# microsoft/mgl

Measured on AMD Instinct MI355X. Metric: GCUPS (+ aligned reads/s) for 150 bp short-read batch, higher is better.
Workload: dtype int16; 1 GPU; BASELINE.json configs[1]: 10000000 Illumina-style 150 bp reads x 256-base reference windows, affine-gap SW, full matrix, GATK params (200,-150,260,11), SOFTCLIP, scores+offset+CIGAR for every pair; pairs_total=10000000, pairs_per_gpu=10000000, target_len=256, query_len=150, input=ascii, parallelism=1 GPU, steps_in_flight=1

## Files before the change

mgl_amd/csrc/sw_capi.cpp:

```cpp
#include "../../include/mgl_sw.h"

#include <hip/hip_runtime.h>

#include <algorithm>
#include <chrono>
#include <cstdint>
#include <cstdio>
#include <functional>
#include <future>
#include <cstring>
#include <mutex>
#include <string>
#include <vector>

#include "sw_ctx_access.h"
#include "sw_device.h"

using namespace mgl_sw_dev;

static_assert(sizeof(mgl_sw_score) == sizeof(Score), "mgl_sw_score layout");

namespace {

constexpr int64_t kDefaultWorkspace = 4ll << 30;
// ... 890 lines not shown
            da.uni_ql = max_ql;
            da.tb = pt.tb;
            da.tb_stride_words = pt.stride;
            da.rec = pt.rec;
            da.scratch = pt.lane ? static_cast<unsigned char *>(ctx->bnd[h].p) : (use_scratch || coop_waves || strip16) ? static_cast<unsigned char *>(ctx->scratch.p) : nullptr;
            da.diag = nullptr;
            da.matrix = d_matrix;
            da.code = d_code;
            da.matrix_lds_offset = 0;
            da.score_only = score_only ? 1 : 0;
            da.grouped = pt.lane && auto_group ? 1 : 0;
            da.strip_k = strip16 ? strip_k : 0;
            da.strip_passes = strip16 ? strip_passes : 0;
            {
                const char *const sce = getenv("MGL_SW_DEBUG_STRIP_CODES");
                da.strip_codes = strip16 && strip_k > 0 && !(sce && atoi(sce) == 0) && strip16_lds_bytes_codes(max_ql, strip_waves) <= 64 * 1024 ? 1 : 0;
            }
            da.fold_k = P.fold.k;
            da.fold_bm = P.fold.bm;
            da.fold_bx = P.fold.bx;
            {
                const char *const wse = getenv("MGL_SW_DEBUG_WALK_STAGED");
                da.walk_staged = wse && atoi(wse) != 0 ? 1 : 0;
            }
            da.lane_slots = 0;
            da.tile_ctr = nullptr;
            da.grid_fault = nullptr;
            da.gate = nullptr;
            da.gate_dev = nullptr;
            da.gate_failed = nullptr;
            da.gate_timeout_ticks = 0;
            if (pt.lane && (lane_ck || da.grouped)) {
                da.lane_slots = (int)std::min<int64_t>(lane_slots - (side && n_parts > 1 ? std::min<int64_t>(side_reserve, lane_slots / 2) : 0), (pt.count + 127) / 128);
                if (ctx->cur_gate && !hooks) {
                    da.gate = ctx->cur_gate;
                    da.gate_dev = ctx->cur_gate_dev;
                    da.gate_failed = reinterpret_cast<int32_t *>(const_cast<int64_t *>(ctx->cur_gate) + 1);
                    da.gate_timeout_ticks = 100000000u;
                    if (const char *const gte = getenv("MGL_SW_DEBUG_GATE_TIMEOUT_TICKS")) da.gate_timeout_ticks = (unsigned)atoll(gte);
                }
                if ((pt.count + 127) / 128 > da.lane_slots) {
                    da.tile_ctr = static_cast<unsigned *>(ctx->tile_ctr.p) + (size_t)(ctx->tile_seq++ % kTileCounters) * kTileCounterWords;
                    void *fault_dev = nullptr;
                    HIP_TRY(ctx, hipHostGetDevicePointer(&fault_dev, ctx->pin_fault, 0));
                    da.grid_fault = static_cast<int32_t *>(fault_dev);
                }
// ... 2029 lines not shown
```

mgl_amd/csrc/sw_device.h:

```cpp
#ifndef MGL_SW_DEVICE_H
#define MGL_SW_DEVICE_H

#include <hip/hip_runtime.h>
#include <stddef.h>
#include <stdint.h>

namespace mgl_sw_dev {

constexpr int NEG_INF = -0x40000000;
constexpr int OS_SOFTCLIP = 1, OS_INDEL = 2, OS_LEAD_ID = 4, OS_IGNORE = 8;
constexpr int ERR_CIGAR_OVERFLOW = 2;
constexpr int ERR_DEVICE = 4;
constexpr int MATRIX_DIM = 32;

struct Score {
    int32_t mqe, mqe_t, max, max_t, max_q, seg_length;
};

struct DpRecord {
    int32_t mqe, mqe_t, max, max_t, max_q, seg;
    int32_t g_tail;
    int32_t sps;
};

// ... 17 lines not shown
};

struct DpArgs {
    SeqSet t, q;
    int64_t first;
    int64_t count;
    int match, mismatch, gopen, gext, strategy;
    int sps_cap;
    int uni_tl, uni_ql;
    uint32_t *tb;
    int64_t tb_stride_words;
    DpRecord *rec;
    unsigned char *scratch;
    unsigned long long *diag;
    const int8_t *matrix;
    const uint8_t *code;
    int matrix_lds_offset;
    int score_only;
    int grouped;
    int strip_k;
    int strip_passes;
    int strip_codes;
    int lane_slots;
    unsigned *tile_ctr;
    int32_t *grid_fault;
    const int64_t *gate;
    int64_t *gate_dev;
    int32_t *gate_failed;
    unsigned gate_timeout_ticks;
    const int32_t *tile_order;
    const int64_t *slot_off;
    int fold_k, fold_bm, fold_bx;
    int walk_staged;
};

struct TbArgs {
    SeqSet t, q;
    int64_t first, count;
    int strategy;
    const uint32_t *tb;
    int64_t tb_stride_words;
    int packed16;
    int rows_per_stripe;
    int uni_ql;
    const DpRecord *rec;
    int32_t *offset;
// ... 243 lines not shown
```

mgl_amd/csrc/sw_dp16_lane_ck.hip:

```cpp
#include <hip/hip_runtime.h>
#include <stdint.h>
#include <stdio.h>
#include <stdlib.h>
#include <string.h>

#include <type_traits>

#include "sw_device.h"
#include "sw_lane_cell.h"
#include "sw_traceback.h"

#ifndef MGL_CK_ABLATE
#define MGL_CK_ABLATE 0
#endif
#if (MGL_CK_ABLATE != 0 || defined(MGL_CK_PHASES) || defined(MGL_CK_TRACE)) && !defined(MGL_VARIANT_BUILD)
#error "MGL_CK_ABLATE / MGL_CK_PHASES are measurement builds (scripts/build_variant.sh defines MGL_VARIANT_BUILD): never the shipped library"
#endif

#ifdef MGL_CK_PHASES
__device__ unsigned long long mgl_ck_phase_ticks[16];
#define CK_PHASE(k)                                                                                    \
    do {                                                                                               \
        const unsigned long long now_ = __builtin_amdgcn_s_memtime();                                  \
        if (lane == 0) atomicAdd(&mgl_ck_phase_ticks[k], now_ - phase_t0);                             \
// ... 52 lines not shown
#pragma unroll
        for (int k = 0; k < W / 4 + 2; ++k) e[k] = (d[k + 2] & by2) | (d[k] & ~by2);
#pragma unroll
        for (int k = 0; k < W / 4 + 1; ++k) w[k] = (e[k + 1] & by1) | (e[k] & ~by1);
        return s & 3u;
    }
};

struct WaveMem {
    uint2 *bnd;
    uint2 *mid;
    unsigned *ck;
    uint4 *blk;
    const uint2 *rows;
    const unsigned *cku;
    const uint32_t *blku;
    const unsigned *seq;
    unsigned mid_off, t_off, lane;
    template <class T>
    __device__ __forceinline__ static T at32(const void *base, unsigned byte_off) { return *reinterpret_cast<const T *>(static_cast<const char *>(base) + byte_off); }
    __device__ __forceinline__ uint2 row16(int m, int ql, int j) const
    {
        return at32<uint2>(rows, 8u * ((m & 1) ? mid_off + (unsigned)(((m >> 1) * ql + j - 1) * 64) + lane : (unsigned)(((m >> 1) * (ql + 1) + j) * 64) + lane));
    }
    __device__ __forceinline__ unsigned qblock(int blk4, int half) const { return at32<unsigned>(seq, 4u * ((unsigned)((2 * blk4 + half) * 64) + lane)); }
    __device__ __forceinline__ unsigned tblock(int blk4, int half) const { return at32<unsigned>(seq, 4u * (t_off + (unsigned)((2 * blk4 + half) * 64) + lane)); }
    __device__ __forceinline__ unsigned flags(int cc, int r4) const { return at32<unsigned>(blku, 4u * ((unsigned)(cc * 256 + r4) + 4u * lane)); }
};

struct WinShift {
    unsigned t, q;
};
struct PathWalk {
    int I, J, pi, pj, n, seg;
    int hc;
    int mode;
    char state;
    bool done;
    bool stuck;
    SeqBlocks ts, qs;
    CigarWriter cw;

    __device__ __forceinline__ void take(char next, int step)
    {
        if (next == state) {
            seg += step;
// ... 165 lines not shown
        }
        return n;
    }
    static constexpr int VB = 4;
    __device__ __forceinline__ WinShift win64_load(const WaveMem &wm, int half, int tblocks, int qblocks, const BlockGeom &g, unsigned (&tw)[17], unsigned (&qw)[17]) const
    {
        WinShift sh;
        if (g.direct) {
            sh.t = ts.window<64>(I, g.tl, tw);
            sh.q = qs.window<64>(J, g.ql, qw);
            return sh;
        }
        const int dt = (I - 64) >> 2, dq = (J - 64) >> 2;
#pragma unroll
        for (int k = 0; k < 17; ++k) {
            tw[k] = wm.tblock(min(max(dt + k, 0), tblocks - 1), half);
            qw[k] = wm.qblock(min(max(dq + k, 0), qblocks - 1), half);
        }
        sh.t = (unsigned)(I - 64) & 3u;
        sh.q = (unsigned)(J - 64) & 3u;
        return sh;
    }
    __device__ __forceinline__ int stretch_to(int m) const { return min(I - max((((I - 1) >> 4) - m) << 4, 0), J); }
    __device__ __forceinline__ void grid_load(const WaveMem &wm, int ql, unsigned (&w)[VB]) const
    {
#pragma unroll
        for (int m = 0; m < VB; ++m) {
            const int L = stretch_to(m), ie = I - L, je = J - L;
            w[m] = wm.row16(ie >> 4, ql, max(je, 1)).x;
        }
    }
    __device__ __forceinline__ bool verify_apply(const unsigned (&tw)[17], const unsigned (&qw)[17], const WinShift sh, const unsigned (&w)[VB], int half,
                                                 const BlockGeom &g)
    {
        if (!can_verify()) return false;
        const unsigned st = sh.t, sq = sh.q;
        unsigned long long differ = 0;
#pragma unroll
        for (int k = 0; k < 16; ++k) {
            const unsigned tt = __builtin_amdgcn_alignbyte(tw[k + 1], tw[k], st);
            const unsigned nz = nonzero_bytes((g.codes ? tt << 3 : tt) ^ __builtin_amdgcn_alignbyte(qw[k + 1], qw[k], sq)) >> 7;
            const unsigned nib = ((nz * 0x08040201u) >> 24) & 0xfu;
            differ |= (unsigned long long)nib << (4 * (15 - k));
        }
        int took = 0, h_at = hc;
        bool all = true;
#pragma unroll
        for (int m = 0; m < VB; ++m) {
            const int L = stretch_to(m), ie = I - L, je = J - L;
            const int he = ie == 0 ? border(je, g.gopen, g.gext, g.indel)
                         : je == 0 ? border(ie, g.gopen, g.gext, g.indel)
                                   : (half ? hi16(w[m]) : lo16(w[m])) - (ie + je) * g.gext - g.base;
// ... 1 lines not shown
            const bool ok = hc - he == L * g.match + __popcll(differ & in) * (g.mismatch - g.match);
            took = ok ? L : took;
            h_at = ok ? he : h_at;
            all = all && ok;
        }
        stuck = !all;
        if (took > 0) {
            take('M', took);
            I -= took;
            J -= took;
            hc = h_at;
            pi = I;
            pj = J;
            done = !(I > 0 && J > 0);
        }
        return all && !done;
    }
    __device__ __forceinline__ int edge_len() const
    {
        if (done || mode != 0 || !stuck) return 0;
        const int lc = J - ((J - 1) & ~(CK - 1));
        return J > CK && lc < stretch_to(0) ? lc : 0;
    }
    __device__ __forceinline__ unsigned edge_load(const WaveMem &wm, int nb, int lc) const
    {
        const int r0 = I - lc - 1, b = (J - 1) / CK;
        return WaveMem::at32<unsigned>(wm.cku, 4u * ((unsigned)((((r0 >> 5) * (nb - 1) + (b - 1)) * 64 + 2 * (r0 & (R - 1))) * 64) + wm.lane));
    }
    __device__ __forceinline__ bool edge_apply(const unsigned w, const unsigned (&tw)[5], const unsigned (&qw)[5], const WinShift sh, int lc, int half,
                                               const BlockGeom &g)
    {
        if (lc == 0) return false;
        const int ie = I - lc, je = J - lc;
        const int he = (half ? hi16(w) : lo16(w)) - (ie + je) * g.gext - g.base;
        if (hc - he != lc * g.match + mismatches(tw, qw, sh, lc, g.codes) * (g.mismatch - g.match)) return false;
        take('M', lc);
        I = ie;
        J = je;
        hc = he;
        pi = I;
        pj = J;
        return true;
    }
    __device__ __forceinline__ void finish(const TbArgs &a, const DpRecord *rp, int64_t o)
    {
        int off;
        if (a.strategy == OS_SOFTCLIP) {
            cw.push_front(state, seg);
            if (J > 0) cw.push_front('S', J);
// ... 31 lines not shown

constexpr int ROW_KEY_MAX_QL = 65536;
__device__ __forceinline__ int row_pref(const int tl, const int ql, const int j)
{
    const int d = abs(tl - j);
    const int nearer = max(min(ql, tl + d - 1) - max(1, tl - d + 1) + 1, 0);
    return ql - 1 - nearer - ((j > tl && tl - d >= 1) ? 1 : 0);
}
__device__ __forceinline__ int row_col(const int tl, const int ql, const int pref)
{
    const int r = ql - 1 - pref;
    if (tl > ql) return ql - r;
    const int m = min(tl - 1, ql - tl);
    if (r <= 2 * m) return (r & 1) ? tl - ((r + 1) >> 1) : tl + (r >> 1);
    return tl - 1 > m ? tl - (r - m) : tl + (r - m);
}

enum : int {
    NOT_LAST = 0,
    LAST_ROW_KEYS = 1,
    LAST_ROW_STORED = 2,
};

template <int LAST, int CODES>
__device__ __forceinline__ void ck_strip(const int k, const int tl, const int ql, const int nb, const WaveMem &wm, const unsigned *qst, const unsigned *tst,
                                         const LaneConsts &c, const int gopen, const int gext, const int base, const bool indel, int &bestA,
                                         int &bestA_i, int &bestB, int &bestB_i, int &keyA, int &keyB, unsigned &corner)
{
    const int i0 = k * R;
    unsigned h[R], f[R], t[R];
#pragma unroll
    for (int r4 = 0; r4 < R / 4; ++r4) {
        const unsigned ta = tst[(size_t)(2 * ((i0 >> 2) + r4)) * 64], tb = tst[(size_t)(2 * ((i0 >> 2) + r4) + 1) * 64];
        t[4 * r4 + 0] = __builtin_amdgcn_perm(tb, ta, 0x0c040c00u) | (CODES ? CODE_SEL : 0u);
        t[4 * r4 + 1] = __builtin_amdgcn_perm(tb, ta, 0x0c050c01u) | (CODES ? CODE_SEL : 0u);
        t[4 * r4 + 2] = __builtin_amdgcn_perm(tb, ta, 0x0c060c02u) | (CODES ? CODE_SEL : 0u);
        t[4 * r4 + 3] = __builtin_amdgcn_perm(tb, ta, 0x0c070c03u) | (CODES ? CODE_SEL : 0u);
    }
#pragma unroll
    for (int r = 0; r < R; ++r) {
        const int row = i0 + r + 1;
        const int hb = border(row, gopen, gext, indel) + row * gext + base;
        h[r] = pack2(hb, hb);
        f[r] = pk_sub(h[r], c.o_e);
    }
    const int rl = tl - 1 - i0;

    const uint2 *bp = wm.bnd + ((size_t)k * (ql + 1) + 1) * 64;
    uint2 *bo = wm.bnd + ((size_t)(k + 1) * (ql + 1) + 1) * 64;
    uint2 *mp = wm.mid + (size_t)k * ql * 64;
    unsigned *ckp = wm.ck + (size_t)k * (nb - 1) * 64 * 64;
    unsigned hd = bp[-64].x;
    int j = 1;
    auto one_column = [&](const uint2 top, const unsigned qa, const unsigned qb, const int u) {
        unsigned e = top.y;
        uint2 mid;
        if (CODES)
            column<R, true, true, CODES>(h, f, t, code_table((qa >> (8 * u)) & 0xffu, c.bm, c.bx), hd, e, c, nullptr, &mid, code_table((qb >> (8 * u)) & 0xffu, c.bm, c.bx));
        else
            column<R, true, true, false>(h, f, t, __builtin_amdgcn_perm(qb, qa, 0x0c040c00u + 0x00010001u * u), hd, e, c, nullptr, &mid);
        hd = top.x;
        if (!(MGL_CK_ABLATE & 4)) mp[0] = mid;
        mp += 64;
        if (LAST == NOT_LAST) {
            bo[0] = make_uint2(h[R - 1], e);
        } else {
            unsigned bot = h[R - 1];
            if (rl != R - 1) {
#pragma unroll
                for (int r = 0; r < R - 1; ++r) bot = (r == rl) ? h[r] : bot;
            }
            if (LAST == LAST_ROW_STORED) {
                bo[0] = make_uint2(bot, 0u);
            } else {
                const int jc = j + u, lift = (ql - jc) * gext;
                const unsigned w = pk_add(bot, pack2(lift, lift)), pref = (unsigned)row_pref(tl, ql, jc);
                keyA = max(keyA, (int)((w << 16) | pref));
                keyB = max(keyB, (int)((w & 0xffff0000u) | pref));
            }
        }
        if (LAST != LAST_ROW_KEYS) bo += 64;
    };
    auto save = [&]() {
#pragma unroll
        for (int r = 0; r < R; ++r) {
            ckp[(size_t)(2 * r) * 64] = h[r];
            ckp[(size_t)(2 * r + 1) * 64] = f[r];
        }
        ckp += 64 * 64;
    };
    uint2 n0 = bp[0], n1 = bp[64], n2 = bp[128], n3 = bp[192];
    unsigned nqa = qst[0], nqb = qst[64];
    for (; j + 3 <= ql; j += 4) {
        if (!(MGL_CK_ABLATE & 2) && j > 1 && ((j - 1) & (CK - 1)) == 0) save();
        const uint2 top0 = n0, top1 = n1, top2 = n2, top3 = n3;
        const unsigned qa = nqa, qb = nqb;
        qst += 128;
        bp += 256;
        n0 = bp[0];
        n1 = bp[64];
        n2 = bp[128];
        n3 = bp[192];
        nqa = qst[0];
        nqb = qst[64];
        one_column(top0, qa, qb, 0);
        one_column(top1, qa, qb, 1);
        one_column(top2, qa, qb, 2);
        one_column(top3, qa, qb, 3);
    }
    if (j <= ql) {
        if (j > 1 && ((j - 1) & (CK - 1)) == 0) save();
        one_column(n0, nqa, nqb, 0);
        if (j + 1 <= ql) one_column(n1, nqa, nqb, 1);
        if (j + 2 <= ql) one_column(n2, nqa, nqb, 2);
    }
    if (LAST != NOT_LAST) {
        corner = h[R - 1];
        if (rl != R - 1) {
#pragma unroll
            for (int r = 0; r < R - 1; ++r) corner = (r == rl) ? h[r] : corner;
        }
    }
#pragma unroll
    for (int r = 0; r < R; ++r) {
        const int row = i0 + r + 1;
        if (row <= tl) {
            const int unshift = -(row + ql) * gext - base;
            const int ca = lo16(h[r]) + unshift, cb = hi16(h[r]) + unshift;
            if (ca >= bestA) {
                bestA = ca;
                bestA_i = row;
            }
            if (cb >= bestB) {
                bestB = cb;
                bestB_i = row;
            }
        }
    }
}

template <int CODES>
__device__ __forceinline__ void ck_block(const int sA, const int bA, const int sB, const int bB, const bool needA, const bool needB, const BlockGeom &g,
                                         const WaveMem &wm, const LaneConsts &c, const int groups = CK / 8)
{
    unsigned h[RB], f[RB], t[RB];
#pragma unroll
    for (int r4 = 0; r4 < RB / 4; ++r4) {
        const unsigned ta = wm.tblock(sA * (RB / 4) + r4, 0), tb = wm.tblock(sB * (RB / 4) + r4, 1);
        t[4 * r4 + 0] = __builtin_amdgcn_perm(tb, ta, 0x0c040c00u) | (CODES ? CODE_SEL : 0u);
        t[4 * r4 + 1] = __builtin_amdgcn_perm(tb, ta, 0x0c050c01u) | (CODES ? CODE_SEL : 0u);
        t[4 * r4 + 2] = __builtin_amdgcn_perm(tb, ta, 0x0c060c02u) | (CODES ? CODE_SEL : 0u);
        t[4 * r4 + 3] = __builtin_amdgcn_perm(tb, ta, 0x0c070c03u) | (CODES ? CODE_SEL : 0u);
    }
    {
        const unsigned ia = (unsigned)((((sA >> 1) * (g.nb - 1) + max(bA - 1, 0)) * 64 + (sA & 1) * 2 * RB) * 64) + wm.lane;
        const unsigned ib = (unsigned)((((sB >> 1) * (g.nb - 1) + max(bB - 1, 0)) * 64 + (sB & 1) * 2 * RB) * 64) + wm.lane;
        unsigned v[2 * RB];
#pragma unroll
        for (int x = 0; x < 2 * RB; ++x) v[x] = 0u;
        if (needA && bA > 0) {
#pragma unroll
            for (int x = 0; x < 2 * RB; ++x) v[x] = WaveMem::at32<unsigned>(wm.cku, 4u * (ia + (unsigned)(x * 64)));
        }
#pragma unroll
        for (int r = 0; r < RB; ++r) {
            const int rowA = sA * RB + r + 1;
            const int fa_ = border(rowA, g.gopen, g.gext, g.indel) + rowA * g.gext + g.base;
            h[r] = bA > 0 ? v[2 * r] : (unsigned)fa_;
            f[r] = bA > 0 ? v[2 * r + 1] : (unsigned)(fa_ - (g.gopen - g.gext));
        }
#pragma unroll
        for (int x = 0; x < 2 * RB; ++x) v[x] = 0u;
        if (needB && bB > 0) {
#pragma unroll
            for (int x = 0; x < 2 * RB; ++x) v[x] = WaveMem::at32<unsigned>(wm.cku, 4u * (ib + (unsigned)(x * 64)));
        }
#pragma unroll
        for (int r = 0; r < RB; ++r) {
            const int rowB = sB * RB + r + 1;
            const int fb_ = border(rowB, g.gopen, g.gext, g.indel) + rowB * g.gext + g.base;
            const unsigned hb = bB > 0 ? v[2 * r] : (unsigned)fb_ << 16, gb = bB > 0 ? v[2 * r + 1] : (unsigned)(fb_ - (g.gopen - g.gext)) << 16;
            h[r] = lo_hi(h[r], hb);
            f[r] = lo_hi(f[r], gb);
        }
    }
    unsigned hd;
    {
        unsigned a0 = 0u, b0 = 0u;
        if (needA) a0 = wm.row16(sA, g.ql, CK * bA).x;
        if (needB) b0 = wm.row16(sB, g.ql, CK * bB).x;
        if (sA & 1) {
            const int row = sA * RB;
            const int v = border(row, g.gopen, g.gext, g.indel) + row * g.gext + g.base;
            a0 = bA > 0 ? a0 : (unsigned)v;
        }
        if (sB & 1) {
            const int row = sB * RB;
            const int v = border(row, g.gopen, g.gext, g.indel) + row * g.gext + g.base;
            b0 = bB > 0 ? b0 : (unsigned)v << 16;
        }
        hd = lo_hi(a0, b0);
    }
    const int qmax = ((g.ql + 3) >> 2) - 1;
#pragma unroll 1
    for (int gg = 0; gg < groups; ++gg) {
        uint2 va[8], vb[8];
#pragma unroll
        for (int u = 0; u < 8; ++u) va[u] = vb[u] = make_uint2(0u, 0u);
        if (needA) {
#pragma unroll
            for (int u = 0; u < 8; ++u) va[u] = wm.row16(sA, g.ql, min(CK * bA + 8 * gg + u + 1, g.ql));
        }
        if (needB) {
#pragma unroll
            for (int u = 0; u < 8; ++u) vb[u] = wm.row16(sB, g.ql, min(CK * bB + 8 * gg + u + 1, g.ql));
        }
        unsigned qa[2], qb[2];
#pragma unroll
        for (int u = 0; u < 2; ++u) {
            qa[u] = wm.qblock(min(bA * (CK / 4) + 2 * gg + u, qmax), 0);
            qb[u] = wm.qblock(min(bB * (CK / 4) + 2 * gg + u, qmax), 1);
        }
#pragma unroll
        for (int u = 0; u < 8; ++u) {
            unsigned e = lo_hi(va[u].y, vb[u].y);
            uint4 *const out = wm.blk + (size_t)(8 * gg + u) * 64;
            if (CODES)
                column<RB, false, false, CODES>(h, f, t, code_table((qa[u >> 2] >> (8 * (u & 3))) & 0xffu, c.bm, c.bx), hd, e, c, out, nullptr,
                                                code_table((qb[u >> 2] >> (8 * (u & 3))) & 0xffu, c.bm, c.bx));
            else
                column<RB, false, false, false>(h, f, t, __builtin_amdgcn_perm(qb[u >> 2], qa[u >> 2], 0x0c040c00u + 0x00010001u * (u & 3)), hd, e, c, out);
            hd = lo_hi(va[u].x, vb[u].x);
        }
    }
}

typedef uint32_t dwords4 __attribute__((ext_vector_type(4), aligned(4)));
__device__ __forceinline__ void seq_words4(const SeqWords &s, const int k0, unsigned (&w)[4])
// ... 86 lines not shown
#pragma unroll
        for (int u = 0; u < 4; ++u) {
            const unsigned va = __builtin_amdgcn_alignbit(wa[u + 1], wa[u], sa.shift), vb = __builtin_amdgcn_alignbit(wb[u + 1], wb[u], sb.shift);
#pragma unroll
            for (int x = 0; x < 4; ++x) {
                const int blk = cb + 4 * u + x;
                if (blk < nblocks) {
                    const unsigned ca = spread_2bit((va >> (8 * x)) & 0xffu), cb2 = spread_2bit((vb >> (8 * x)) & 0xffu);
                    dst[(size_t)(2 * blk) * 64] = QUERY ? ca << 3 : ca;
                    dst[(size_t)(2 * blk + 1) * 64] = QUERY ? cb2 << 3 : cb2;
                }
            }
        }
    }
}

__device__ __forceinline__ void lds_to_global(void *dst, const unsigned char *src, const int bytes, const int lane)
{
    const int whole = bytes & ~15;
    for (int k = lane * 16; k < whole; k += 1024) *reinterpret_cast<uint4 *>(static_cast<unsigned char *>(dst) + k) = *reinterpret_cast<const uint4 *>(src + k);
    for (int k = whole + lane * 4; k < bytes; k += 256) *reinterpret_cast<unsigned *>(static_cast<unsigned char *>(dst) + k) = *reinterpret_cast<const unsigned *>(src + k);
}

template <bool VIA_LDS, bool FOLD>
__device__ __forceinline__ void sw_dp16_lane_ck_tile(const DpArgs &a, const TbArgs &walk_in, const int64_t gw, const int64_t slot, const int lane, unsigned char *out_lds, const bool first)
{
    const int64_t n_ls = (a.count + 1) >> 1;
#ifdef MGL_CK_PHASES
    unsigned long long phase_t0 = __builtin_amdgcn_s_memtime();
#endif
    const int64_t ls = gw * 64 + lane;
    const bool lvalid = ls < n_ls;
    const int64_t slotA = lvalid ? 2 * ls : a.count - 1;
    const bool validB = lvalid && (2 * ls + 1 < a.count);
    const int64_t slotB = validB ? 2 * ls + 1 : slotA;

    const bool grouped = a.grouped != 0;
    const int tl = grouped ? __builtin_amdgcn_readfirstlane(a.t.length(a.first + gw * 128)) : a.uni_tl;
    const int ql = grouped ? __builtin_amdgcn_readfirstlane(a.q.length(a.first + gw * 128)) : a.uni_ql;
    const int match = a.match, gopen = a.gopen, gext = a.gext;
    const bool indel = (a.strategy & (OS_INDEL | OS_LEAD_ID)) != 0;
    const int base = dp16_base(tl, ql, match, gext);
    LaneConsts c;
    c.delta = pack2(a.mismatch - match, a.mismatch - match);
    c.one = pack2(1, 1);
    c.o_e = pack2(gopen - gext, gopen - gext);
    c.k2 = pack2(match + 2 * gext, match + 2 * gext);
// ... 43 lines not shown
                stage_ascii<true, true>(a.q.data + a.q.off[pA], a.q.data + a.q.off[pB], ql, qblocks, qst);
            } else {
                stage_ascii<false, false>(a.t.data + a.t.off[pA], a.t.data + a.t.off[pB], tl, tblocks, tst);
                stage_ascii<false, true>(a.q.data + a.q.off[pA], a.q.data + a.q.off[pB], ql, qblocks, qst);
            }
        }
        if (grouped || first) {
            for (int j = 0; j <= ql; ++j) {
                const int hb0 = border(j, gopen, gext, indel) + j * gext + base;
                const unsigned hp = pack2(hb0, hb0);
                wm.bnd[(size_t)j * 64] = make_uint2(hp, pk_sub(hp, c.o_e));
            }
            for (int k = 1; k <= strips; ++k) {
                const int hb0 = border(k * R, gopen, gext, indel) + k * R * gext + base;
                wm.bnd[(size_t)k * (ql + 1) * 64] = make_uint2(pack2(hb0, hb0), 0u);
            }
        }
    }

    CK_PHASE(0);
    int bestA = NEG_INF, bestA_i = -1, bestB = NEG_INF, bestB_i = -1;
    int keyA = INT32_MIN, keyB = INT32_MIN;
    unsigned corner = 0u;
    const bool row_stored = ql > ROW_KEY_MAX_QL;
#define CK_STRIPS(CMP)                                                                                                                      \
    do {                                                                                                                                    \
        for (int k = 0; k < strips - 1; ++k)                                                                                                \
            ck_strip<NOT_LAST, CMP>(k, tl, ql, nb, wm, qst, tst, c, gopen, gext, base, indel, bestA, bestA_i, bestB, bestB_i, keyA, keyB, corner); \
        if (row_stored)                                                                                                                     \
            ck_strip<LAST_ROW_STORED, CMP>(strips - 1, tl, ql, nb, wm, qst, tst, c, gopen, gext, base, indel, bestA, bestA_i, bestB, bestB_i, keyA, keyB, corner); \
        else                                                                                                                                \
            ck_strip<LAST_ROW_KEYS, CMP>(strips - 1, tl, ql, nb, wm, qst, tst, c, gopen, gext, base, indel, bestA, bestA_i, bestB, bestB_i, keyA, keyB, corner); \
    } while (0)
    if (codes)
        CK_STRIPS(CM);
    else
        CK_STRIPS(CMP_BYTES);
#undef CK_STRIPS

    CK_PHASE(1);
    int rmA, rdA, rjA, rmB, rdB, rjB;
    const int frame = (tl + ql) * gext + base;
    const int cornerA = lo16(corner) - frame, cornerB = hi16(corner) - frame;
    if (!row_stored) {
        rjA = row_col(tl, ql, keyA & 0xffff);
        rjB = row_col(tl, ql, keyB & 0xffff);
        rmA = (keyA >> 16) - frame;
        rmB = (keyB >> 16) - frame;
        rdA = abs(tl - rjA);
        rdB = abs(tl - rjB);
    } else {
        rmA = rmB = NEG_INF;
        rdA = rjA = rdB = rjB = 0x7fffffff;
        const uint2 *const last = wm.bnd + (size_t)strips * (ql + 1) * 64;
        for (int j0 = 1; j0 <= ql; j0 += 8) {
// ... 65 lines not shown
    BlockGeom &geom = geom_launch;
    geom.tl = tl;
    geom.ql = ql;
    geom.nb = nb;
    geom.match = match;
    geom.mismatch = a.mismatch;
    geom.gopen = gopen;
    geom.gext = gext;
    geom.base = base;
    geom.indel = indel;
    geom.codes = codes;
    geom.direct = false;
    const bool by_score = !(MGL_CK_ABLATE & 8);
    const int tblocks = strips * (R / 4), qblocks = (ql + 3) >> 2;
    auto stretches = [&](auto direct_form) __attribute__((always_inline)) {
        BlockGeom geom = geom_launch;
        geom.direct = decltype(direct_form)::value;
        geom.codes = !decltype(direct_form)::value && codes;
        for (;;) {
            unsigned ta[17], qa[17], tb[17], qb[17], ga[PathWalk::VB], gb[PathWalk::VB];
            WinShift sa = {0u, 0u}, sb = {0u, 0u};
            if (wa.can_verify()) {
                sa = wa.win64_load(wm, 0, tblocks, qblocks, geom, ta, qa);
                wa.grid_load(wm, ql, ga);
            }
            if (wb.can_verify()) {
                sb = wb.win64_load(wm, 1, tblocks, qblocks, geom, tb, qb);
                wb.grid_load(wm, ql, gb);
            }
            const bool ma = wa.verify_apply(ta, qa, sa, ga, 0, geom), mb = wb.verify_apply(tb, qb, sb, gb, 1, geom);
#ifdef MGL_CK_PHASES
            if (lane == 0) atomicAdd(&mgl_ck_phase_ticks[12], 1ull);
#endif
            if (!__builtin_amdgcn_ballot_w64(ma || mb)) break;
        }
        {
            const int ea = wa.edge_len(), eb = wb.edge_len();
            if (__builtin_amdgcn_ballot_w64((ea | eb) != 0)) {
                unsigned ta[5], qa[5], tb[5], qb[5], ha = 0u, hb = 0u;
                WinShift sa = {0u, 0u}, sb = {0u, 0u};
                if (ea) {
                    sa = wa.win_load(wm, 0, tblocks, qblocks, geom, ta, qa);
                    ha = wa.edge_load(wm, nb, ea);
                }
                if (eb) {
                    sb = wb.win_load(wm, 1, tblocks, qblocks, geom, tb, qb);
                    hb = wb.edge_load(wm, nb, eb);
                }
                const bool xa = wa.edge_apply(ha, ta, qa, sa, ea, 0, geom), xb = wb.edge_apply(hb, tb, qb, sb, eb, 1, geom);
#ifdef MGL_CK_PHASES
                const unsigned long long took_ = __popcll(__builtin_amdgcn_ballot_w64(xa)) + __popcll(__builtin_amdgcn_ballot_w64(xb));
                const unsigned long long tried_ = __popcll(__builtin_amdgcn_ballot_w64(ea != 0)) + __popcll(__builtin_amdgcn_ballot_w64(eb != 0));
                if (lane == 0) {
                    atomicAdd(&mgl_ck_phase_ticks[10], took_);
                    atomicAdd(&mgl_ck_phase_ticks[11], tried_ - took_);
                }
#else
                (void)xa;
                (void)xb;
#endif
            }
        }
    };
    auto block_walk = [&](auto direct_form, const int kA, const int bA, const int kB, const int bB) __attribute__((always_inline)) {
        BlockGeom geom = geom_launch;
        geom.direct = decltype(direct_form)::value;
        geom.codes = !decltype(direct_form)::value && codes;
        for (;;) {
            const bool la = wa.can_load(kA, bA), lb = wb.can_load(kB, bB);
            unsigned fa[PathWalk::LOOK], fb[PathWalk::LOOK], ta[5], qa[5], tb[5], qb[5];
// ... 5 lines not shown
            if (lb) {
                wb.load(wm, fb);
                if (wb.mode == 0) sb = wb.win_load(wm, 1, tblocks, qblocks, geom, tb, qb);
            }
            const bool ga = wa.apply(fa, ta, qa, sa, 0, kA, bA, geom), gb = wb.apply(fb, tb, qb, sb, 1, kB, bB, geom);
            if (!__builtin_amdgcn_ballot_w64(ga || gb)) break;
        }
    };
    while (!(MGL_CK_ABLATE & 1) && __builtin_amdgcn_ballot_w64(!wa.done || !wb.done) != 0) {
        if (by_score) {
            if (direct)
                stretches(std::true_type{});
            else
                stretches(std::false_type{});
            CK_PHASE(3);
            if (__builtin_amdgcn_ballot_w64(!wa.done || !wb.done) == 0) break;
        }
        const int kA = max(wa.pi - 1, 0) >> 4, bA = max(wa.pj - 1, 0) / CK, kB = max(wb.pi - 1, 0) >> 4, bB = max(wb.pj - 1, 0) / CK;
        int reach = max(!wa.done ? (max(wa.pj - 1, 0) % CK) + 1 : 0, !wb.done ? (max(wb.pj - 1, 0) % CK) + 1 : 0);
#pragma unroll
        for (int m = 32; m >= 1; m >>= 1) reach = max(reach, __shfl_xor(reach, m));
        const int groups = __builtin_amdgcn_readfirstlane((reach + 7) >> 3);
        if (codes)
            ck_block<CM>(kA, bA, kB, bB, !wa.done, !wb.done, geom, wm, c, groups);
        else
            ck_block<CMP_BYTES>(kA, bA, kB, bB, !wa.done, !wb.done, geom, wm, c, groups);
        asm volatile("s_waitcnt vmcnt(0)" ::: "memory");
        CK_PHASE(4);
#ifdef MGL_CK_PHASES
        if (lane == 0) atomicAdd(&mgl_ck_phase_ticks[8], 1ull);
#endif
        if (direct)
            block_walk(std::true_type{}, kA, bA, kB, bB);
        else
            block_walk(std::false_type{}, kA, bA, kB, bB);
        wa.stuck = wb.stuck = false;
        CK_PHASE(5);
    }
    CK_PHASE(6);
    if (lvalid) wa.finish(walk, a.rec + slotA, oA);
    if (validB) wb.finish(walk, a.rec + slotB, oB);
    if (via_lds) {
        __builtin_amdgcn_fence(__ATOMIC_RELEASE, "workgroup");
        __builtin_amdgcn_wave_barrier();
        __builtin_amdgcn_fence(__ATOMIC_ACQUIRE, "workgroup");
        const int64_t p0 = a.first + gw * 128;
        const int np = (int)min((int64_t)128, a.count - gw * 128);
        lds_to_global(walk_in.cigar + (size_t)p0 * walk_in.cigar_stride, out_lds, np * walk_in.cigar_stride, lane);
        if (walk_in.score) lds_to_global(walk_in.score + p0, l_score, np * 24, lane);
        lds_to_global(walk_in.offset + p0, l_off, np * 4, lane);
        if (walk_in.cigar_len) lds_to_global(walk_in.cigar_len + p0, l_len, np * 4, lane);
        if (walk_in.status) lds_to_global(walk_in.status + p0, l_status, np * 4, lane);
        __builtin_amdgcn_wave_barrier();
    }
    CK_PHASE(7);
#ifdef MGL_CK_PHASES
    if (lane == 0) atomicAdd(&mgl_ck_phase_ticks[9], 1ull);
#endif
}

}

template <bool VIA_LDS, bool FOLD>
__device__ __forceinline__ void lane_ck_grid(const DpArgs &a, const TbArgs &walk, unsigned char *out_lds)
{
    const int lane = threadIdx.x & 63;
    const int64_t tiles = (((a.count + 1) >> 1) + 63) >> 6, slots = gridDim.x, slot = blockIdx.x;
    unsigned long long diag_t0 = 0, diag_w0 = 0;
    if (a.diag) {
        diag_t0 = __builtin_amdgcn_s_memtime();
        diag_w0 = __builtin_amdgcn_s_memrealtime();
    }
    int64_t arrived = a.gate ? 0 : INT64_MAX;
    unsigned long long *const ctr = reinterpret_cast<unsigned long long *>(a.tile_ctr);
    for (int64_t tile = slot; tile < tiles;) {
        if (arrived < a.first + min(a.count, (tile + 2) * 128)) {
            const int64_t need = a.first + min(a.count, (tile + 2) * 128);
            int lo = 0, hi = 0, flags = 0;
            if (lane == 0) {
                unsigned long long since = __builtin_amdgcn_s_memrealtime();
                long long last = arrived, seen;
                for (;;) {
                    seen = (long long)__hip_atomic_load(reinterpret_cast<const unsigned long long *>(a.gate_dev), __ATOMIC_RELAXED, __HIP_MEMORY_SCOPE_AGENT);
                    if (seen >= need || seen < 0) break;
                    const unsigned long long now = __builtin_amdgcn_s_memrealtime();
                    const unsigned long long polled = __hip_atomic_load(reinterpret_cast<const unsigned long long *>(a.gate_dev) + 1, __ATOMIC_RELAXED, __HIP_MEMORY_SCOPE_AGENT);
// ... 17 lines not shown
                        break;
                    }
                    __builtin_amdgcn_s_sleep(32);
                }
                lo = (int)(unsigned)(unsigned long long)seen;
                hi = (int)(unsigned)((unsigned long long)seen >> 32);
            }
            lo = __builtin_amdgcn_readfirstlane(lo);
            hi = __builtin_amdgcn_readfirstlane(hi);
            flags = __builtin_amdgcn_readfirstlane(flags);
            arrived = (int64_t)((unsigned long long)(unsigned)lo | (unsigned long long)(unsigned)hi << 32);
            if (flags & 1) {
                if (lane == 0) __hip_atomic_store(a.gate_failed, 1, __ATOMIC_RELAXED, __HIP_MEMORY_SCOPE_SYSTEM);
                break;
            }
            if (arrived < 0) break;
#ifndef MGL_CK_NO_GATE_FENCE
            __builtin_amdgcn_fence(__ATOMIC_ACQUIRE, "agent");
#endif
        }
#ifdef MGL_CK_TRACE
        const unsigned long long t0 = __builtin_amdgcn_s_memrealtime();
#endif
        sw_dp16_lane_ck_tile<VIA_LDS, FOLD>(a, walk, tile, slot, lane, out_lds, tile == slot);
#ifdef MGL_CK_TRACE
        if (lane == 0 && tile < (1 << 17)) {
            unsigned hw;
            asm volatile("s_getreg_b32 %0, hwreg(HW_REG_HW_ID)" : "=s"(hw));
            unsigned xcc;
            asm volatile("s_getreg_b32 %0, hwreg(HW_REG_XCC_ID)" : "=s"(xcc));
            mgl_ck_trace[4 * tile + 0] = (unsigned long long)slot;
            mgl_ck_trace[4 * tile + 1] = (unsigned long long)hw | (unsigned long long)(xcc & 15u) << 32;
            mgl_ck_trace[4 * tile + 2] = t0;
            mgl_ck_trace[4 * tile + 3] = __builtin_amdgcn_s_memrealtime();
        }
#endif
        if (tiles <= slots) break;
        unsigned next = 0;
        if (lane == 0) {
            next = (unsigned)__hip_atomic_fetch_add(ctr, 1ull, __ATOMIC_RELAXED, __HIP_MEMORY_SCOPE_AGENT);
            if (next >= (unsigned)tiles && a.grid_fault) __hip_atomic_store(a.grid_fault, 1, __ATOMIC_RELAXED, __HIP_MEMORY_SCOPE_SYSTEM);
        }
        tile = slots + (int64_t)(unsigned)__builtin_amdgcn_readfirstlane((int)next);
    }
    if (tiles > slots && lane == 0) {
        const unsigned out = (unsigned)(__hip_atomic_fetch_add(ctr, 1ull << 32, __ATOMIC_RELAXED, __HIP_MEMORY_SCOPE_AGENT) >> 32);
        if (out == (unsigned)slots - 1u) {
            __hip_atomic_store(ctr, 0ull, __ATOMIC_RELAXED, __HIP_MEMORY_SCOPE_AGENT);
        } else if (out >= (unsigned)slots && a.grid_fault) {
            __hip_atomic_store(a.grid_fault, 1, __ATOMIC_RELAXED, __HIP_MEMORY_SCOPE_SYSTEM);
        }
    }
    if (a.diag && lane == 0) {
        a.diag[2 * slot] = __builtin_amdgcn_s_memtime() - diag_t0;
        a.diag[2 * slot + 1] = __builtin_amdgcn_s_memrealtime() - diag_w0;
    }
}

__global__ __launch_bounds__(64, 2) void sw_dp16_lane_ck_kernel(const DpArgs a, const TbArgs walk)
{
    __shared__ __attribute__((aligned(16))) unsigned char out_lds[LANE_CK_OUT_LDS_BYTES];
    lane_ck_grid<true, false>(a, walk, out_lds);
}

__global__ __launch_bounds__(64, 2) void sw_dp16_lane_ck_scatter_kernel(const DpArgs a, const TbArgs walk) { lane_ck_grid<false, false>(a, walk, nullptr); }

__global__ __launch_bounds__(64, 2) void sw_dp16_lane_ck_kernel_fold(const DpArgs a, const TbArgs walk)
{
    __shared__ __attribute__((aligned(16))) unsigned char out_lds[LANE_CK_OUT_LDS_BYTES];
    lane_ck_grid<true, true>(a, walk, out_lds);
}
__global__ __launch_bounds__(64, 2) void sw_dp16_lane_ck_scatter_kernel_fold(const DpArgs a, const TbArgs walk) { lane_ck_grid<false, true>(a, walk, nullptr); }

bool lane16_ck_supported(const SeqSet &t, const SeqSet &q) { return (t.packed2 != 0) == (q.packed2 != 0); }

hipError_t launch_dp16_lane_ck(const DpArgs &a, const TbArgs &walk, hipStream_t stream)
{
    const int64_t tiles = ((a.count + 1) / 2 + 63) / 64;
    if (a.lane_slots < 1 || (tiles > a.lane_slots && !a.tile_ctr)) return hipErrorInvalidValue;
    const dim3 grid((unsigned)(tiles < a.lane_slots ? tiles : a.lane_slots)), block(64);
    if (walk.coalesced_out)
        hipLaunchKernelGGL(a.fold_k ? sw_dp16_lane_ck_kernel_fold : sw_dp16_lane_ck_kernel, grid, block, 0, stream, a, walk);
    else
        hipLaunchKernelGGL(a.fold_k ? sw_dp16_lane_ck_scatter_kernel_fold : sw_dp16_lane_ck_scatter_kernel, grid, block, 0, stream, a, walk);
    return hipGetLastError();
}

}

#ifdef MGL_CK_TRACE
extern "C" int mgl_ck_trace_dump(const char *path)
{
    static unsigned long long h[4 << 17];
    hipDeviceSynchronize();
    if (hipMemcpyFromSymbol(h, HIP_SYMBOL(mgl_ck_trace), sizeof h) != hipSuccess) return 1;
    FILE *f = fopen(path, "wb");
    if (!f) return 2;
    fwrite(h, 1, sizeof h, f);
    fclose(f);
    memset(h, 0, sizeof h);
    hipMemcpyToSymbol(HIP_SYMBOL(mgl_ck_trace), h, sizeof h);
    return 0;
}
#endif

#ifdef MGL_CK_PHASES
extern "C" void mgl_ck_phases_dump()
// ... 16 lines not shown
```

Before: 6946 GCUPS.

## Store checkpoint and mid-row state in narrow delta-compressed layout for fold kernels

```diff
diff --git a/mgl_amd/csrc/sw_capi.cpp b/mgl_amd/csrc/sw_capi.cpp
--- a/mgl_amd/csrc/sw_capi.cpp
+++ b/mgl_amd/csrc/sw_capi.cpp
@@ -936,6 +936,10 @@
             {
                 const char *const wse = getenv("MGL_SW_DEBUG_WALK_STAGED");
                 da.walk_staged = wse && atoi(wse) != 0 ? 1 : 0;
+            }
+            {
+                const char *const cwe = getenv("MGL_SW_DEBUG_CK_WIDE");
+                da.ck_wide = cwe && atoi(cwe) != 0 ? 1 : 0;
             }
             da.lane_slots = 0;
             da.tile_ctr = nullptr;
diff --git a/mgl_amd/csrc/sw_device.h b/mgl_amd/csrc/sw_device.h
--- a/mgl_amd/csrc/sw_device.h
+++ b/mgl_amd/csrc/sw_device.h
@@ -63,6 +63,7 @@
     int strip_passes;
     int strip_codes;
     int lane_slots;
+    int ck_wide;
     unsigned *tile_ctr;
     int32_t *grid_fault;
     const int64_t *gate;
diff --git a/mgl_amd/csrc/sw_dp16_lane_ck.hip b/mgl_amd/csrc/sw_dp16_lane_ck.hip
--- a/mgl_amd/csrc/sw_dp16_lane_ck.hip
+++ b/mgl_amd/csrc/sw_dp16_lane_ck.hip
@@ -98,6 +98,33 @@
     __device__ __forceinline__ uint2 row16(int m, int ql, int j) const
     {
         return at32<uint2>(rows, 8u * ((m & 1) ? mid_off + (unsigned)(((m >> 1) * ql + j - 1) * 64) + lane : (unsigned)(((m >> 1) * (ql + 1) + j) * 64) + lane));
+    }
+    __device__ __forceinline__ static bool mid_tail_wide(int ql, int j) { return ((j - 1) >> 2) == (ql >> 2) && (ql & 3) != 3; }
+    template <bool NARROW>
+    __device__ __forceinline__ unsigned mid_byte_off(int strip, int ql, int j) const
+    {
+        if (!NARROW) return 8u * (mid_off + (unsigned)((strip * ql + j - 1) * 64) + lane);
+        const int c = j - 1;
+        const unsigned group = 8u * mid_off + (unsigned)(strip * ql * 512 + (c >> 2) * 1536);
+        return group + (mid_tail_wide(ql, j) ? (unsigned)((c & 3) * 512) + 8u * lane : (unsigned)((c & 3) * 4) + 16u * lane);
+    }
+    template <bool NARROW>
+    __device__ __forceinline__ unsigned row16_h(int m, int ql, int j) const
+    {
+        if (!NARROW) return row16(m, ql, j).x;
+        return at32<unsigned>(rows, (m & 1) ? mid_byte_off<true>(m >> 1, ql, j) : 8u * ((unsigned)(((m >> 1) * (ql + 1) + j) * 64) + lane));
+    }
+    template <bool NARROW>
+    __device__ __forceinline__ uint2 row16_n(int m, int ql, int j) const
+    {
+        if (!NARROW) return row16(m, ql, j);
+        const int c = j - 1;
+        const bool bytes = (m & 1) != 0 && !mid_tail_wide(ql, j);
+        const unsigned hoff = (m & 1) ? mid_byte_off<true>(m >> 1, ql, j) : 8u * ((unsigned)(((m >> 1) * (ql + 1) + j) * 64) + lane);
+        const unsigned soff = bytes ? 8u * mid_off + (unsigned)((m >> 1) * ql * 512 + (c >> 2) * 1536 + 1024 + ((c >> 1) & 1) * 4) + 8u * lane : hoff + 4u;
+        const unsigned hv = at32<unsigned>(rows, hoff), sv = at32<unsigned>(rows, soff);
+        const unsigned d = __builtin_amdgcn_perm(0u, sv, (c & 1) ? 0x0c030c02u : 0x0c010c00u);
+        return make_uint2(hv, bytes ? pk_sub(hv, d) : sv);
     }
     __device__ __forceinline__ unsigned qblock(int blk4, int half) const { return at32<unsigned>(seq, 4u * ((unsigned)((2 * blk4 + half) * 64) + lane)); }
     __device__ __forceinline__ unsigned tblock(int blk4, int half) const { return at32<unsigned>(seq, 4u * (t_off + (unsigned)((2 * blk4 + half) * 64) + lane)); }
@@ -309,12 +336,13 @@
         return sh;
     }
     __device__ __forceinline__ int stretch_to(int m) const { return min(I - max((((I - 1) >> 4) - m) << 4, 0), J); }
+    template <bool NARROW>
     __device__ __forceinline__ void grid_load(const WaveMem &wm, int ql, unsigned (&w)[VB]) const
     {
 #pragma unroll
         for (int m = 0; m < VB; ++m) {
             const int L = stretch_to(m), ie = I - L, je = J - L;
-            w[m] = wm.row16(ie >> 4, ql, max(je, 1)).x;
+            w[m] = wm.row16_h<NARROW>(ie >> 4, ql, max(je, 1));
         }
     }
     __device__ __forceinline__ bool verify_apply(const unsigned (&tw)[17], const unsigned (&qw)[17], const WinShift sh, const unsigned (&w)[VB], int half,
@@ -362,9 +390,12 @@
         const int lc = J - ((J - 1) & ~(CK - 1));
         return J > CK && lc < stretch_to(0) ? lc : 0;
     }
+    template <bool NARROW>
     __device__ __forceinline__ unsigned edge_load(const WaveMem &wm, int nb, int lc) const
     {
         const int r0 = I - lc - 1, b = (J - 1) / CK;
+        if (NARROW)
+            return WaveMem::at32<unsigned>(wm.cku, (unsigned)(((r0 >> 5) * (nb - 1) + (b - 1)) * 16384 + ((r0 & (R - 1)) >> 2) * 1024 + (r0 & 3) * 4) + 16u * wm.lane);
         return WaveMem::at32<unsigned>(wm.cku, 4u * ((unsigned)((((r0 >> 5) * (nb - 1) + (b - 1)) * 64 + 2 * (r0 & (R - 1))) * 64) + wm.lane));
     }
     __device__ __forceinline__ bool edge_apply(const unsigned w, const unsigned (&tw)[5], const unsigned (&qw)[5], const WinShift sh, int lc, int half,
@@ -442,7 +473,7 @@
     LAST_ROW_STORED = 2,
 };
 
-template <int LAST, int CODES>
+template <int LAST, int CODES, bool NARROW>
 __device__ __forceinline__ void ck_strip(const int k, const int tl, const int ql, const int nb, const WaveMem &wm, const unsigned *qst, const unsigned *tst,
                                          const LaneConsts &c, const int gopen, const int gext, const int base, const bool indel, int &bestA,
                                          int &bestA_i, int &bestB, int &bestB_i, int &keyA, int &keyB, unsigned &corner)
@@ -469,6 +500,11 @@
     const uint2 *bp = wm.bnd + ((size_t)k * (ql + 1) + 1) * 64;
     uint2 *bo = wm.bnd + ((size_t)(k + 1) * (ql + 1) + 1) * 64;
     uint2 *mp = wm.mid + (size_t)k * ql * 64;
+    char *mg = reinterpret_cast<char *>(const_cast<uint2 *>(wm.rows)) + (size_t)8 * wm.mid_off + (size_t)k * ql * 512;
+    char *cg = reinterpret_cast<char *>(const_cast<unsigned *>(wm.cku)) + (size_t)k * (nb - 1) * 16384;
+    const unsigned l16 = 16u * wm.lane, l8 = 8u * wm.lane;
+    unsigned mh[4] = {0u, 0u, 0u, 0u}, md0 = 0u, md[2] = {0u, 0u};
+    unsigned me[2] = {0u, 0u};
     unsigned *ckp = wm.ck + (size_t)k * (nb - 1) * 64 * 64;
     unsigned hd = bp[-64].x;
     int j = 1;
@@ -480,8 +516,18 @@
         else
             column<R, true, true, false>(h, f, t, __builtin_amdgcn_perm(qb, qa, 0x0c040c00u + 0x00010001u * u), hd, e, c, nullptr, &mid);
         hd = top.x;
-        if (!(MGL_CK_ABLATE & 4)) mp[0] = mid;
-        mp += 64;
+        if (NARROW) {
+            mh[u] = mid.x;
+            if (u < 2) me[u] = mid.y;
+            const unsigned d = pk_sub(mid.x, mid.y);
+            if (u & 1)
+                md[u >> 1] = __builtin_amdgcn_perm(d, md0, 0x06040200u);
+            else
+                md0 = d;
+        } else {
+            if (!(MGL_CK_ABLATE & 4)) mp[0] = mid;
+            mp += 64;
+        }
         if (LAST == NOT_LAST) {
             bo[0] = make_uint2(h[R - 1], e);
         } else {
@@ -501,13 +547,37 @@
         }
         if (LAST != LAST_ROW_KEYS) bo += 64;
     };
+    auto mid_group = [&](const int cols) {
+        if (cols == 3) md[1] = __builtin_amdgcn_perm(md0, md0, 0x06040200u);
+        if (!(MGL_CK_ABLATE & 4)) {
+            *reinterpret_cast<uint4 *>(mg + l16) = make_uint4(mh[0], mh[1], mh[2], mh[3]);
+            *reinterpret_cast<uint2 *>(mg + 1024 + l8) = make_uint2(md[0], md[1]);
+        }
+        mg += 1536;
+    };
     auto save = [&]() {
-#pragma unroll
-        for (int r = 0; r < R; ++r) {
-            ckp[(size_t)(2 * r) * 64] = h[r];
-            ckp[(size_t)(2 * r + 1) * 64] = f[r];
-        }
-        ckp += 64 * 64;
+        if (NARROW) {
+#pragma unroll
+            for (int x = 0; x < R / 4; ++x) *reinterpret_cast<uint4 *>(cg + x * 1024 + l16) = make_uint4(h[4 * x], h[4 * x + 1], h[4 * x + 2], h[4 * x + 3]);
+#pragma unroll
+            for (int x = 0; x < R / 8; ++x) {
+                unsigned d[4];
+#pragma unroll
+                for (int y = 0; y < 4; ++y) {
+                    const int r = 8 * x + 2 * y;
+                    d[y] = __builtin_amdgcn_perm(pk_sub(h[r + 1], f[r + 1]), pk_sub(h[r], f[r]), 0x06040200u);
+                }
+                *reinterpret_cast<uint4 *>(cg + (R / 4 + x) * 1024 + l16) = make_uint4(d[0], d[1], d[2], d[3]);
+            }
+            cg += 16384;
+        } else {
+#pragma unroll
+            for (int r = 0; r < R; ++r) {
+                ckp[(size_t)(2 * r) * 64] = h[r];
+                ckp[(size_t)(2 * r + 1) * 64] = f[r];
+            }
+            ckp += 64 * 64;
+        }
     };
     uint2 n0 = bp[0], n1 = bp[64], n2 = bp[128], n3 = bp[192];
     unsigned nqa = qst[0], nqb = qst[64];
@@ -527,12 +597,21 @@
         one_column(top1, qa, qb, 1);
         one_column(top2, qa, qb, 2);
         one_column(top3, qa, qb, 3);
+        if (NARROW) mid_group(4);
     }
     if (j <= ql) {
         if (j > 1 && ((j - 1) & (CK - 1)) == 0) save();
         one_column(n0, nqa, nqb, 0);
         if (j + 1 <= ql) one_column(n1, nqa, nqb, 1);
         if (j + 2 <= ql) one_column(n2, nqa, nqb, 2);
+        if (NARROW) {
+            if (j + 2 <= ql) {
+                mid_group(3);
+            } else if (!(MGL_CK_ABLATE & 4)) {
+                *reinterpret_cast<uint2 *>(mg + l8) = make_uint2(mh[0], me[0]);
+                if (j + 1 <= ql) *reinterpret_cast<uint2 *>(mg + 512 + l8) = make_uint2(mh[1], me[1]);
+            }
+        }
     }
     if (LAST != NOT_LAST) {
         corner = h[R - 1];
@@ -559,7 +638,7 @@
     }
 }
 
-template <int CODES>
+template <int CODES, bool NARROW>
 __device__ __forceinline__ void ck_block(const int sA, const int bA, const int sB, const int bB, const bool needA, const bool needB, const BlockGeom &g,
                                          const WaveMem &wm, const LaneConsts &c, const int groups = CK / 8)
 {
@@ -576,11 +655,40 @@
         const unsigned ia = (unsigned)((((sA >> 1) * (g.nb - 1) + max(bA - 1, 0)) * 64 + (sA & 1) * 2 * RB) * 64) + wm.lane;
         const unsigned ib = (unsigned)((((sB >> 1) * (g.nb - 1) + max(bB - 1, 0)) * 64 + (sB & 1) * 2 * RB) * 64) + wm.lane;
         unsigned v[2 * RB];
+        auto load_narrow = [&](const int s, const int b) {
+            const unsigned off = (unsigned)(((s >> 1) * (g.nb - 1) + max(b - 1, 0)) * 16384 + (s & 1) * 4096) + 16u * wm.lane;
+            uint4 hv[RB / 4], dv[RB / 8];
+#pragma unroll
+            for (int x = 0; x < RB / 4; ++x) hv[x] = WaveMem::at32<uint4>(wm.cku, off + (unsigned)(x * 1024));
+#pragma unroll
+            for (int x = 0; x < RB / 8; ++x) dv[x] = WaveMem::at32<uint4>(wm.cku, off + (unsigned)(8192 - (s & 1) * 2048 + x * 1024));
+#pragma unroll
+            for (int x = 0; x < RB / 4; ++x) {
+                v[8 * x + 0] = hv[x].x;
+                v[8 * x + 2] = hv[x].y;
+                v[8 * x + 4] = hv[x].z;
+                v[8 * x + 6] = hv[x].w;
+            }
+#pragma unroll
+            for (int x = 0; x < RB / 8; ++x) {
+                const unsigned d[4] = {dv[x].x, dv[x].y, dv[x].z, dv[x].w};
+#pragma unroll
+                for (int y = 0; y < 4; ++y) {
+                    const int r = 8 * x + 2 * y;
+                    v[2 * r + 1] = pk_sub(v[2 * r], __builtin_amdgcn_perm(0u, d[y], 0x0c010c00u));
+                    v[2 * r + 3] = pk_sub(v[2 * r + 2], __builtin_amdgcn_perm(0u, d[y], 0x0c030c02u));
+                }
+            }
+        };
 #pragma unroll
         for (int x = 0; x < 2 * RB; ++x) v[x] = 0u;
         if (needA && bA > 0) {
-#pragma unroll
-            for (int x = 0; x < 2 * RB; ++x) v[x] = WaveMem::at32<unsigned>(wm.cku, 4u * (ia + (unsigned)(x * 64)));
+            if (NARROW) {
+                load_narrow(sA, bA);
+            } else {
+#pragma unroll
+                for (int x = 0; x < 2 * RB; ++x) v[x] = WaveMem::at32<unsigned>(wm.cku, 4u * (ia + (unsigned)(x * 64)));
+            }
         }
 #pragma unroll
         for (int r = 0; r < RB; ++r) {
@@ -592,8 +700,12 @@
 #pragma unroll
         for (int x = 0; x < 2 * RB; ++x) v[x] = 0u;
         if (needB && bB > 0) {
-#pragma unroll
-            for (int x = 0; x < 2 * RB; ++x) v[x] = WaveMem::at32<unsigned>(wm.cku, 4u * (ib + (unsigned)(x * 64)));
+            if (NARROW) {
+                load_narrow(sB, bB);
+            } else {
+#pragma unroll
+                for (int x = 0; x < 2 * RB; ++x) v[x] = WaveMem::at32<unsigned>(wm.cku, 4u * (ib + (unsigned)(x * 64)));
+            }
         }
 #pragma unroll
         for (int r = 0; r < RB; ++r) {
@@ -607,8 +719,8 @@
     unsigned hd;
     {
         unsigned a0 = 0u, b0 = 0u;
-        if (needA) a0 = wm.row16(sA, g.ql, CK * bA).x;
-        if (needB) b0 = wm.row16(sB, g.ql, CK * bB).x;
+        if (needA) a0 = wm.row16_h<NARROW>(sA, g.ql, CK * bA);
+        if (needB) b0 = wm.row16_h<NARROW>(sB, g.ql, CK * bB);
         if (sA & 1) {
             const int row = sA * RB;
             const int v = border(row, g.gopen, g.gext, g.indel) + row * g.gext + g.base;
@@ -629,11 +741,11 @@
         for (int u = 0; u < 8; ++u) va[u] = vb[u] = make_uint2(0u, 0u);
         if (needA) {
 #pragma unroll
-            for (int u = 0; u < 8; ++u) va[u] = wm.row16(sA, g.ql, min(CK * bA + 8 * gg + u + 1, g.ql));
+            for (int u = 0; u < 8; ++u) va[u] = wm.row16_n<NARROW>(sA, g.ql, min(CK * bA + 8 * gg + u + 1, g.ql));
         }
         if (needB) {
 #pragma unroll
-            for (int u = 0; u < 8; ++u) vb[u] = wm.row16(sB, g.ql, min(CK * bB + 8 * gg + u + 1, g.ql));
+            for (int u = 0; u < 8; ++u) vb[u] = wm.row16_n<NARROW>(sB, g.ql, min(CK * bB + 8 * gg + u + 1, g.ql));
         }
         unsigned qa[2], qb[2];
 #pragma unroll
@@ -766,7 +878,7 @@
     for (int k = whole + lane * 4; k < bytes; k += 256) *reinterpret_cast<unsigned *>(static_cast<unsigned char *>(dst) + k) = *reinterpret_cast<const unsigned *>(src + k);
 }
 
-template <bool VIA_LDS, bool FOLD>
+template <bool VIA_LDS, bool FOLD, bool NARROW>
 __device__ __forceinline__ void sw_dp16_lane_ck_tile(const DpArgs &a, const TbArgs &walk_in, const int64_t gw, const int64_t slot, const int lane, unsigned char *out_lds, const bool first)
 {
     const int64_t n_ls = (a.count + 1) >> 1;
@@ -856,15 +968,15 @@
     int bestA = NEG_INF, bestA_i = -1, bestB = NEG_INF, bestB_i = -1;
     int keyA = INT32_MIN, keyB = INT32_MIN;
     unsigned corner = 0u;
-    const bool row_stored = ql > ROW_KEY_MAX_QL;
+    const bool row_stored = !NARROW && ql > ROW_KEY_MAX_QL;
 #define CK_STRIPS(CMP)                                                                                                                      \
     do {                                                                                                                                    \
         for (int k = 0; k < strips - 1; ++k)                                                                                                \
-            ck_strip<NOT_LAST, CMP>(k, tl, ql, nb, wm, qst, tst, c, gopen, gext, base, indel, bestA, bestA_i, bestB, bestB_i, keyA, keyB, corner); \
+            ck_strip<NOT_LAST, CMP, NARROW>(k, tl, ql, nb, wm, qst, tst, c, gopen, gext, base, indel, bestA, bestA_i, bestB, bestB_i, keyA, keyB, corner); \
         if (row_stored)                                                                                                                     \
-            ck_strip<LAST_ROW_STORED, CMP>(strips - 1, tl, ql, nb, wm, qst, tst, c, gopen, gext, base, indel, bestA, bestA_i, bestB, bestB_i, keyA, keyB, corner); \
+            ck_strip<LAST_ROW_STORED, CMP, NARROW>(strips - 1, tl, ql, nb, wm, qst, tst, c, gopen, gext, base, indel, bestA, bestA_i, bestB, bestB_i, keyA, keyB, corner); \
         else                                                                                                                                \
-            ck_strip<LAST_ROW_KEYS, CMP>(strips - 1, tl, ql, nb, wm, qst, tst, c, gopen, gext, base, indel, bestA, bestA_i, bestB, bestB_i, keyA, keyB, corner); \
+            ck_strip<LAST_ROW_KEYS, CMP, NARROW>(strips - 1, tl, ql, nb, wm, qst, tst, c, gopen, gext, base, indel, bestA, bestA_i, bestB, bestB_i, keyA, keyB, corner); \
     } while (0)
     if (codes)
         CK_STRIPS(CM);
@@ -976,11 +1088,11 @@
             WinShift sa = {0u, 0u}, sb = {0u, 0u};
             if (wa.can_verify()) {
                 sa = wa.win64_load(wm, 0, tblocks, qblocks, geom, ta, qa);
-                wa.grid_load(wm, ql, ga);
+                wa.template grid_load<NARROW>(wm, ql, ga);
             }
             if (wb.can_verify()) {
                 sb = wb.win64_load(wm, 1, tblocks, qblocks, geom, tb, qb);
-                wb.grid_load(wm, ql, gb);
+                wb.template grid_load<NARROW>(wm, ql, gb);
             }
             const bool ma = wa.verify_apply(ta, qa, sa, ga, 0, geom), mb = wb.verify_apply(tb, qb, sb, gb, 1, geom);
 #ifdef MGL_CK_PHASES
@@ -995,11 +1107,11 @@
                 WinShift sa = {0u, 0u}, sb = {0u, 0u};
                 if (ea) {
                     sa = wa.win_load(wm, 0, tblocks, qblocks, geom, ta, qa);
-                    ha = wa.edge_load(wm, nb, ea);
+                    ha = wa.template edge_load<NARROW>(wm, nb, ea);
                 }
                 if (eb) {
                     sb = wb.win_load(wm, 1, tblocks, qblocks, geom, tb, qb);
-                    hb = wb.edge_load(wm, nb, eb);
+                    hb = wb.template edge_load<NARROW>(wm, nb, eb);
                 }
                 const bool xa = wa.edge_apply(ha, ta, qa, sa, ea, 0, geom), xb = wb.edge_apply(hb, tb, qb, sb, eb, 1, geom);
 #ifdef MGL_CK_PHASES
@@ -1051,9 +1163,9 @@
         for (int m = 32; m >= 1; m >>= 1) reach = max(reach, __shfl_xor(reach, m));
         const int groups = __builtin_amdgcn_readfirstlane((reach + 7) >> 3);
         if (codes)
-            ck_block<CM>(kA, bA, kB, bB, !wa.done, !wb.done, geom, wm, c, groups);
+            ck_block<CM, NARROW>(kA, bA, kB, bB, !wa.done, !wb.done, geom, wm, c, groups);
         else
-            ck_block<CMP_BYTES>(kA, bA, kB, bB, !wa.done, !wb.done, geom, wm, c, groups);
+            ck_block<CMP_BYTES, NARROW>(kA, bA, kB, bB, !wa.done, !wb.done, geom, wm, c, groups);
         asm volatile("s_waitcnt vmcnt(0)" ::: "memory");
         CK_PHASE(4);
 #ifdef MGL_CK_PHASES
@@ -1090,7 +1202,7 @@
 
 }
 
-template <bool VIA_LDS, bool FOLD>
+template <bool VIA_LDS, bool FOLD, bool NARROW>
 __device__ __forceinline__ void lane_ck_grid(const DpArgs &a, const TbArgs &walk, unsigned char *out_lds)
 {
     const int lane = threadIdx.x & 63;
@@ -1154,7 +1266,7 @@
 #ifdef MGL_CK_TRACE
         const unsigned long long t0 = __builtin_amdgcn_s_memrealtime();
 #endif
-        sw_dp16_lane_ck_tile<VIA_LDS, FOLD>(a, walk, tile, slot, lane, out_lds, tile == slot);
+        sw_dp16_lane_ck_tile<VIA_LDS, FOLD, NARROW>(a, walk, tile, slot, lane, out_lds, tile == slot);
 #ifdef MGL_CK_TRACE
         if (lane == 0 && tile < (1 << 17)) {
             unsigned hw;
@@ -1192,17 +1304,23 @@
 __global__ __launch_bounds__(64, 2) void sw_dp16_lane_ck_kernel(const DpArgs a, const TbArgs walk)
 {
     __shared__ __attribute__((aligned(16))) unsigned char out_lds[LANE_CK_OUT_LDS_BYTES];
-    lane_ck_grid<true, false>(a, walk, out_lds);
-}
-
-__global__ __launch_bounds__(64, 2) void sw_dp16_lane_ck_scatter_kernel(const DpArgs a, const TbArgs walk) { lane_ck_grid<false, false>(a, walk, nullptr); }
+    lane_ck_grid<true, false, false>(a, walk, out_lds);
+}
+
+__global__ __launch_bounds__(64, 2) void sw_dp16_lane_ck_scatter_kernel(const DpArgs a, const TbArgs walk) { lane_ck_grid<false, false, false>(a, walk, nullptr); }
 
 __global__ __launch_bounds__(64, 2) void sw_dp16_lane_ck_kernel_fold(const DpArgs a, const TbArgs walk)
 {
     __shared__ __attribute__((aligned(16))) unsigned char out_lds[LANE_CK_OUT_LDS_BYTES];
-    lane_ck_grid<true, true>(a, walk, out_lds);
-}
-__global__ __launch_bounds__(64, 2) void sw_dp16_lane_ck_scatter_kernel_fold(const DpArgs a, const TbArgs walk) { lane_ck_grid<false, true>(a, walk, nullptr); }
+    lane_ck_grid<true, true, true>(a, walk, out_lds);
+}
+__global__ __launch_bounds__(64, 2) void sw_dp16_lane_ck_scatter_kernel_fold(const DpArgs a, const TbArgs walk) { lane_ck_grid<false, true, true>(a, walk, nullptr); }
+__global__ __launch_bounds__(64, 2) void sw_dp16_lane_ck_kernel_fold_wide(const DpArgs a, const TbArgs walk)
+{
+    __shared__ __attribute__((aligned(16))) unsigned char out_lds[LANE_CK_OUT_LDS_BYTES];
+    lane_ck_grid<true, true, false>(a, walk, out_lds);
+}
+__global__ __launch_bounds__(64, 2) void sw_dp16_lane_ck_scatter_kernel_fold_wide(const DpArgs a, const TbArgs walk) { lane_ck_grid<false, true, false>(a, walk, nullptr); }
 
 bool lane16_ck_supported(const SeqSet &t, const SeqSet &q) { return (t.packed2 != 0) == (q.packed2 != 0); }
 
@@ -1211,10 +1329,13 @@
     const int64_t tiles = ((a.count + 1) / 2 + 63) / 64;
     if (a.lane_slots < 1 || (tiles > a.lane_slots && !a.tile_ctr)) return hipErrorInvalidValue;
     const dim3 grid((unsigned)(tiles < a.lane_slots ? tiles : a.lane_slots)), block(64);
+    const int o_e = a.gopen - a.gext;
+    const bool narrow = !a.ck_wide && o_e >= 0 && o_e <= 255 && a.uni_ql <= ROW_KEY_MAX_QL;
     if (walk.coalesced_out)
-        hipLaunchKernelGGL(a.fold_k ? sw_dp16_lane_ck_kernel_fold : sw_dp16_lane_ck_kernel, grid, block, 0, stream, a, walk);
+        hipLaunchKernelGGL(!a.fold_k ? sw_dp16_lane_ck_kernel : narrow ? sw_dp16_lane_ck_kernel_fold : sw_dp16_lane_ck_kernel_fold_wide, grid, block, 0, stream, a, walk);
     else
-        hipLaunchKernelGGL(a.fold_k ? sw_dp16_lane_ck_scatter_kernel_fold : sw_dp16_lane_ck_scatter_kernel, grid, block, 0, stream, a, walk);
+        hipLaunchKernelGGL(!a.fold_k ? sw_dp16_lane_ck_scatter_kernel : narrow ? sw_dp16_lane_ck_scatter_kernel_fold : sw_dp16_lane_ck_scatter_kernel_fold_wide, grid, block, 0,
+                           stream, a, walk);
     return hipGetLastError();
 }
 
```

Result: faster. 7215 GCUPS (median of 6 runs) (+3.9%).
